# mbitsnbites/himg

Measured on AMD Instinct MI355X. Metric: Mpixels/s encode+decode, 4K RGBA q=50, higher is better.
Workload: dtype u8/i16/i32 integer

## Files before the change

himg_amd/csrc/himg_dev.h:

```cpp
#ifndef HIMG_DEV_H_
#define HIMG_DEV_H_

#include <hip/hip_runtime.h>
#include <stdint.h>

namespace himg_dev {

constexpr int kNumSym = 261;
constexpr int kHistStride = 264;
constexpr int kLresSpan = 16384;
constexpr int kIterSyms = 4096;
constexpr int kTreeStride = 384;
constexpr int kMaxCodeLen = 32;
constexpr int kHeadLen = 175;

struct Geom {
  int W, H, C, stride;
  int rows, cols, mrows, mcols;
  int chan_size, lres_size;
  int row_block;
  int ycbcr;
  int lres_spans;
  int use_blocks;
  int fix_t2;
// ... 105 lines not shown
static_assert(kRowTabWords % 4 == 0, "whole 16-byte words");

constexpr int kLresMemoWords = 6;
constexpr int kRecHdr = 72;
constexpr int kRecWin = 8;
struct DecWs {
  DecFrame *frames;
  uint32_t *nodes;
  uint2 *grp;
  uint32_t *gyc;
  uint2 *sub;
  uint32_t *row_off;
  uint32_t *row_len;
  uint8_t *lres_sym;         size_t lres_stride;
  uint8_t *fres_sym;         size_t fres_stride;
  uint8_t *low;              size_t plane_stride;
  uint32_t *lane_start;
  uint32_t *lane_off;
  uint32_t *lane_q;
  uint32_t *parse_stats;
  uint32_t *stats;
  uint32_t *rc_stats;
  int lres_chunks;
  uint32_t *spec_start;
  uint32_t *spec_endpos;
  uint32_t *spec_cnt;
  uint32_t *spec_memo;
  uint64_t *spec_end;
  uint64_t *fix_end;
  uint64_t *spec_tot;
  uint64_t *ver_base;
  int32_t *ver_ok;
  uint64_t *lres_endbit;
};


struct Profiler;

bool enc_uses_row_tokens(const Geom &g, int batch);
int enc_tok_seg(const Geom &g);
inline bool enc_tok_stage_fits(const Geom &g) { return tok_stage_need(g.row_block, enc_tok_seg(g)) <= kTokStage; }
void launch_tok_expand(const Geom &g, const EncWs &ws, int frame, uint8_t *dst, hipStream_t stream);

void launch_encode(const Geom &g, const EncWs &ws, int batch, const uint8_t *d_frames,
                   uint8_t *d_out, size_t out_stride, uint32_t *d_sizes,
                   const StaticChunks &sc, const ShiftTables &st, const LresTables &lt,
                   const uint8_t *d_fmap_lut, hipStream_t stream, Profiler *prof,
                   hipStream_t side, hipEvent_t ev_fork, hipEvent_t ev_join);

void enc_fill_qual_tab(const StaticChunks &sc, const ShiftTables &st, const LresTables &lt, QualTab *qt);
void launch_encode_q(const Geom &g, const EncWs &ws, int batch, const uint8_t *d_frames,
                     uint8_t *d_out, size_t out_stride, uint32_t *d_sizes,
                     const StaticChunks &sc, const QualSel &qs,
                     const uint8_t *d_fmap_lut, hipStream_t stream, Profiler *prof,
                     hipStream_t side, hipEvent_t ev_fork, hipEvent_t ev_join);
struct BudgetState {
  int32_t *quality;
  const uint32_t *budget;
  int32_t *lo, *hi;
  int32_t *state;
  int32_t *err;
};
enum { kBudgetSearch = 0, kBudgetFound = 1, kBudgetTooSmall = 2, kBudgetError = 3 };
void launch_budget_step(const BudgetState &bs, const EncWs &ws, int batch, int probe, int probes, int qmin, int qmax,
                        const uint32_t *d_sizes, int32_t *d_quality, hipStream_t stream, Profiler *prof);
void launch_budget_finish(const BudgetState &bs, const EncWs &ws, int batch, uint32_t *d_sizes, int32_t *d_status,
// ... 109 lines not shown
```

himg_amd/csrc/himg_hip.hip:

```cpp
#include "himg_hip.h"

#include <hip/hip_runtime.h>

#include <cmath>
#include <cstdio>
#include <cstdlib>
#include <cstring>
#include <string>
#include <vector>

#include "himg_dev.h"
#include "himg_tables.h"

using namespace himg_dev;

namespace himg_dev {

struct Profiler {
  bool enabled = false;
  struct Rec { const char *name; hipEvent_t a, b; };
  std::vector<Rec> pending;
  struct Acc { std::string name; double ms = 0; int n = 0; };
  std::vector<Acc> acc;
  const char *cur = nullptr;
// ... 505 lines not shown
      !ctx->d_grp.reserve((size_t)batch * 2 * (1u << kLutBits) * 8) ||
      !ctx->d_gyc.reserve((size_t)batch * 2 * (1u << kLutBits) * 4) ||
      !ctx->d_sub.reserve((size_t)batch * 2 * kSubEntries * 8) ||
      !ctx->d_lane.reserve((size_t)batch * g.rows * (2 * kDecThreads + himg_dev::kRecHdr + (region || himg_dev::dec_rows_fit_lds(g) ? 0 : 6 * kDecThreads)) * 4) ||
      !ctx->d_rows.reserve((size_t)batch * g.rows * 4 * 2) || !ctx->d_lres.reserve(lres * batch) ||
      (!region && !ctx->d_fres.reserve(fres * batch)) || !ctx->d_planes.reserve(plane * batch) ||
      !ctx->d_sizes.reserve((size_t)batch * (region ? 12 : 4)) ||
      !ctx->d_stats.reserve(((size_t)batch * (g.rows + 1) * 8 + (size_t)batch * 4 + (size_t)batch * g.rows * 8) * 4))
    return fail(ctx, HIMG_ERR_HIP, "decoder workspace allocation failed");
  w.frames = (DecFrame *)ctx->d_frames.p;
  w.nodes = (uint32_t *)ctx->d_nodes.p;
  w.grp = (uint2 *)ctx->d_grp.p;
  w.gyc = (uint32_t *)ctx->d_gyc.p;
  w.sub = (uint2 *)ctx->d_sub.p;
  w.lane_start = head_only ? nullptr : (uint32_t *)ctx->d_lane.p;
  w.lane_off = head_only ? nullptr : w.lane_start + (size_t)batch * g.rows * kDecThreads;
  w.lane_q = (head_only || region || himg_dev::dec_rows_fit_lds(g)) ? nullptr : w.lane_off + (size_t)batch * g.rows * (kDecThreads + himg_dev::kRecHdr);
  w.row_off = head_only ? nullptr : (uint32_t *)ctx->d_rows.p;
  w.row_len = head_only ? nullptr : w.row_off + (size_t)batch * g.rows;
  w.lres_sym = (uint8_t *)ctx->d_lres.p; w.lres_stride = lres;
  w.fres_sym = (head_only || region) ? nullptr : (uint8_t *)ctx->d_fres.p; w.fres_stride = (head_only || region) ? 0 : fres;
  w.low = (uint8_t *)ctx->d_planes.p; w.plane_stride = plane;
  w.stats = (uint32_t *)ctx->d_stats.p;
  w.parse_stats = w.stats + (size_t)batch * (g.rows + 1) * 8;
  w.rc_stats = head_only ? nullptr : w.parse_stats + (size_t)batch * 4;
  {
    const size_t max_bits = 8ull * ((size_t)g.lres_size + kTreeStride);
    const size_t cb = (size_t)kDecThreads * kLresSubBits;
    int nch = (int)((max_bits + cb - 1) / cb);
    if (nch > 1024) nch = 1024;
    w.lres_chunks = nch;
    size_t off = 0;
    auto carve = [&](size_t bytes) { size_t o = off; off += round_up(bytes, 256); return o; };
    const size_t o_ss = carve((size_t)batch * nch * kDecThreads * 4);
    const size_t o_sc = carve((size_t)batch * nch * kDecThreads * 4);
    const size_t o_se = carve((size_t)batch * nch * 8);
    const size_t o_st = carve((size_t)batch * nch * 8);
    const size_t o_sp = carve((size_t)batch * nch * kDecThreads * 4);
    const size_t o_fe = carve((size_t)batch * nch * 8);
    const size_t o_vb = carve((size_t)batch * nch * 8);
    const size_t o_ok = carve((size_t)batch * 4);
    const size_t o_eb = carve((size_t)batch * 8);
    const size_t o_mm = carve((size_t)batch * nch * kDecThreads * 4 * himg_dev::kLresMemoWords);
    if (!ctx->d_spec.reserve(off)) return fail(ctx, HIMG_ERR_HIP, "decoder workspace allocation failed");
    uint8_t *b = (uint8_t *)ctx->d_spec.p;
    w.spec_start = (uint32_t *)(b + o_ss); w.spec_cnt = (uint32_t *)(b + o_sc);
    w.spec_end = (uint64_t *)(b + o_se); w.spec_tot = (uint64_t *)(b + o_st);
    w.spec_endpos = (uint32_t *)(b + o_sp); w.fix_end = (uint64_t *)(b + o_fe);
    w.ver_base = (uint64_t *)(b + o_vb); w.ver_ok = (int32_t *)(b + o_ok);
    w.lres_endbit = (uint64_t *)(b + o_eb);
    w.spec_memo = (uint32_t *)(b + o_mm);
  }
  ctx->dec_geom = g;
  ctx->dec_batch = batch;
  ctx->dec_valid = true;
  return HIMG_OK;
}

static std::string format_message(int32_t st) {
  static const char *kStage[] = {"", "Not a RIFF HIMG file.\n", "Error decoding header.\n",
                                 "Error decoding low-res mapping function.\n",
                                 "Error decoding low-res data.\n",
                                 "Error decoding quantization configuration.\n",
                                 "Error decoding full-res mapping function.\n",
                                 "Error decoding full-res data.\n"};
  std::string m;
  if (st & 0x100) m += "Error: Invalid Huffman data.\n";
  const int stage = (st >> 4) & 7;
  m += kStage[stage];
  return m;
}

static int status_to_code(int32_t st) {
  st &= 15;
  switch (st) {
    case 0: return HIMG_OK;
    case 1: return HIMG_ERR_ARG;
    case 3: return HIMG_ERR_UNSUPPORTED;
// ... 1875 lines not shown
```

himg_amd/csrc/kernels_dec.hip:

```cpp
#include "himg_dev.h"
#include "loop_counts.h"

#include <cstdlib>
#include <type_traits>

namespace himg_dev {

__device__ static constexpr uint8_t kScanD[64] = {
    0,  1,  9,  8,  16, 17, 18, 10, 2,  3,  11, 19, 27, 26, 25, 24,
    32, 33, 34, 35, 36, 28, 20, 12, 4,  5,  13, 21, 29, 37, 45, 44,
    43, 42, 41, 40, 48, 49, 50, 51, 52, 53, 54, 46, 38, 30, 22, 14,
    6,  7,  15, 23, 31, 39, 47, 55, 63, 62, 61, 60, 59, 58, 57, 56};

__device__ static constexpr uint8_t kInvScanD[64] = {
    0, 1, 8, 9, 24, 25, 48, 49, 3, 2, 7, 10, 23, 26, 47, 50, 4, 5, 6, 11, 22, 27, 46, 51, 15, 14, 13, 12, 21, 28, 45, 52, 16, 17, 18, 19, 20, 29, 44, 53, 35, 34, 33, 32, 31, 30, 43, 54, 36, 37, 38, 39, 40, 41, 42, 55, 63, 62, 61, 60, 59, 58, 57, 56};

constexpr int kStGeom = 1, kStUnsupported = 3, kStFormat = 4;
__device__ __host__ constexpr int fmt_err(int stage, int huff) { return kStFormat | (stage << 4) | (huff << 8); }
constexpr int kMaxDepth = 32;
constexpr int kMaxNodes = 2 * kNumSym - 1;
constexpr int kMaxSlow = 128;

__device__ __forceinline__ int clamp255d(int x) { return x < 0 ? 0 : (x > 255 ? 255 : x); }

// ... 2333 lines not shown
}

template <bool FAST>
__global__ __launch_bounds__(256) void k_sse(Geom g, const uint8_t *frames, const uint8_t *fres_sym, size_t fres_stride,
                                             const uint8_t *rec, size_t plane_stride, const SseTab *tabs,
                                             const int32_t *quality, unsigned long long *sse) {
  __shared__ __attribute__((aligned(16))) uint32_t s_tab[kRowTabWords];
  __shared__ unsigned long long s_part[4];
  const int v = blockIdx.y, f = blockIdx.z, tid = threadIdx.x;
  const int q = __builtin_amdgcn_readfirstlane(
      ((const __attribute__((address_space(4))) int32_t *)(uintptr_t)quality)[f]);
  if (tid < kRowTabWords / 4) reinterpret_cast<uint4 *>(s_tab)[tid] = reinterpret_cast<const uint4 *>(tabs[q].w)[tid];
  __syncthreads();
  const int16_t *s_unmap = reinterpret_cast<const int16_t *>(s_tab);
  const uint8_t *s_shift = reinterpret_cast<const uint8_t *>(s_tab + 128);
  const uint32_t *s_shiftp = s_tab + 160;
  const int it = blockIdx.x * 256 + tid;
  uint32_t acc = 0;
  if (pair_tile(it) < g.cols)
    acc = transform_store_pair<(FAST ? -1 : 0), FAST, true>(
        g, g.cols, fres_sym + (size_t)f * fres_stride + (size_t)v * g.row_block, rec + (size_t)f * plane_stride,
        s_unmap, s_shift, s_shiftp, g.ycbcr, pair_tile(it), pair_half(it), v, nullptr, nullptr, true, false, 0,
        frames + (size_t)f * (size_t)g.frame_bytes, g.stride);
#pragma unroll
  for (int d = 32; d >= 1; d >>= 1) acc += __shfl_xor(acc, d);
  if ((tid & 63) == 0) s_part[tid >> 6] = acc;
  __syncthreads();
  if (tid == 0) {
    const unsigned long long t = s_part[0] + s_part[1] + s_part[2] + s_part[3];
    if (t) __hip_atomic_fetch_add(sse + f, t, __ATOMIC_RELAXED, __HIP_MEMORY_SCOPE_AGENT);
  }
}

template <int COLS, bool TENS = false>
__device__ __forceinline__ void dec_row_fused_body(const Geom &g, const DecWs &ws, const uint8_t *packed,
                                                   size_t in_stride, const uint32_t *sizes,
                                                   uint8_t *out_frames, int r0, int r1, int rpw,
                                                   const int bx, const int f, const int gx, const int gy,
                                                   const uint32_t next_lin, const bool again, const bool same_tables,
                                                   TensK td = nullptr) {
  extern __shared__ __attribute__((aligned(16))) uint8_t smem[];
  if (COLS == 512) rpw = 1;
  const FusedLayout L = fused_layout(g.row_block, rpw);
  const uint32_t rb16 = ((uint32_t)g.row_block + 15u) & ~15u;
  uint8_t *sym0 = smem + L.sym;
  LdsTables &T = *reinterpret_cast<LdsTables *>(smem + L.tab);
  StreamShared *sh = reinterpret_cast<StreamShared *>(smem + L.sh);
  int16_t *s_unmap = reinterpret_cast<int16_t *>(smem + L.unmap);
  uint8_t *s_shift = smem + L.shift;
  uint32_t *s_shiftp = reinterpret_cast<uint32_t *>(smem + L.shiftp);

  int tid_ = threadIdx.x;
  asm volatile("" : "+v"(tid_));
  __builtin_assume(tid_ >= 0 && tid_ < kDecThreads);
  const int tid = tid_;
  const long long c_in = clock64();
  DecFrame *df = ws.frames + f;
  const uint8_t *low = ws.low + (size_t)f * ws.plane_stride;
  PreLane pl = {};
  uint32_t pre_lr[4] = {0, 0, 0, 0}, pre_off0 = 0, pre_len0 = 0;
  if constexpr (COLS == 512) {
    const size_t ri = (size_t)f * g.rows + (size_t)(r0 + bx);
    const uint32_t *ps = ws.lane_start + ri * kDecThreads, *po = ws.lane_off + ri * (kDecThreads + kRecHdr);
    pl.start = ps[tid]; pl.off = po[tid]; pl.nxt = po[tid + 1];
    pl.nstart = tid + 1 < kDecThreads ? ps[tid + 1] : ~0u;
    pl.tot = po[kDecThreads]; pl.endrel = po[kDecThreads + 1]; pl.valid = po[kDecThreads + 2]; pl.rounds = po[kDecThreads + 3];
    pre_off0 = ws.row_off[ri]; pre_len0 = ws.row_len[ri];
    const int u = pair_tile(tid), hs = pair_half(tid), v = r0 + bx;
    const int u2 = min(u + 1, COLS - 1), v2 = min(v + 1, g.rows - 1);
    const uint32_t pstride = (uint32_t)g.rows * COLS, o1 = (uint32_t)v * COLS, o2 = (uint32_t)v2 * COLS;
#pragma unroll
    for (int cc = 0; cc < 2; ++cc) {
      const uint32_t m = (uint32_t)(2 * hs + cc) * pstride;
// ... 26 lines not shown
  const int rb = r0 + bx * rpw;
  const int nr = COLS == 512 ? 1 : min(rpw, r1 - rb);
  if (COLS == 512 && again) __syncthreads();
  {
    uint4 z;
    z.x = z.y = z.z = z.w = 0;
    const int n16 = (int)(rb16 >> 4) * nr;
    for (int k = tid; k < n16; k += kDecThreads) reinterpret_cast<uint4 *>(sym0)[k] = z;
  }
  if (ld_tab) {
    reinterpret_cast<uint4 *>(T.grp)[tid] = t_grp;
    if (tid < kRowTabWords / 4) reinterpret_cast<uint4 *>(smem + L.unmap)[tid] = t_row;
    if (tid < kSubEntries / 2) reinterpret_cast<uint4 *>(T.grp + (1 << kLutBits))[tid] = t_sub;
    if (tid < kMaxNodes + 1) T.nd[tid] = t_nd;
  }
  if constexpr (COLS == 512) {
    if (tid == 0) { sh->flag = st0; sh->err = 0; sh->endbit = ~0ull; }
  }
  __syncthreads();
  if constexpr (COLS == 512) {
    if (sh->flag) return;
  }

  auto decode_row = [&](int i) {
    const int r = rb + i;
    if (tid == 0) {
      uint32_t *st = ws.stats + ((size_t)f * (g.rows + 1) + r + 1) * 8;
      st[2] = 0; st[3] = 0;
    }
    if constexpr (COLS == 512) {
      uint32_t *st = ws.stats + ((size_t)f * (g.rows + 1) + r + 1) * 8;
      const int rc = decode_row_recorded(p, sizes[f], pre_off0, pre_len0, (uint32_t)g.row_block, tb, sh, sym0, st, pl);
      if (rc >= 0) return rc;
      return decode_stream_fused_cold(p, sizes[f], pre_off0, pre_len0, (uint32_t)g.row_block,
                                      reinterpret_cast<const uint32_t *>(tb.grp), tb.nd, sh, sym0, st,
                                      (uint32_t)g.max_sub, (uint32_t)g.lead_bits);
    }
    const size_t ri = (size_t)f * g.rows + (size_t)r;
    const uint32_t *ps = ws.lane_start + ri * kDecThreads, *po = ws.lane_off + ri * (kDecThreads + kRecHdr);
    PreLane q;
    q.start = ps[tid]; q.off = po[tid]; q.nxt = po[tid + 1];
    q.nstart = tid + 1 < kDecThreads ? ps[tid + 1] : ~0u;
    q.tot = po[kDecThreads]; q.endrel = po[kDecThreads + 1]; q.valid = po[kDecThreads + 2]; q.rounds = po[kDecThreads + 3];
    const uint32_t off_r = ws.row_off[ri], len_r = ws.row_len[ri];
    if (i > 0) __syncthreads();
    if (tid == 0) { sh->err = 0; sh->endbit = ~0ull; }
    __syncthreads();
    uint32_t *st = ws.stats + ((size_t)f * (g.rows + 1) + r + 1) * 8;
    const int rc = decode_row_recorded(p, sizes[f], off_r, len_r, (uint32_t)g.row_block, tb, sh, sym0 + (size_t)i * rb16, st, q);
    if (rc >= 0) return rc;
    return decode_stream_fused_cold(p, sizes[f], off_r, len_r, (uint32_t)g.row_block,
                                    reinterpret_cast<const uint32_t *>(tb.grp), tb.nd, sh, sym0 + (size_t)i * rb16, st,
                                    (uint32_t)g.max_sub, (uint32_t)g.lead_bits);
  };
  int bad = 0;
  if constexpr (COLS == 512) {
    bad = decode_row(0);
  } else {
#pragma unroll 1
    for (int i = 0; i < nr && !bad; ++i) bad = decode_row(i);
  }
  if (bad) {
    if (tid == 0) atomicMax(&df->status, fmt_err(7, 1));
    return;
  }

  const long long c_p2 = clock64();
  uint32_t pf_a = 0;
  bool pf_on = false;
  {
    const int fn = (int)(next_lin / (uint32_t)gx), rn = r0 + (int)(next_lin % (uint32_t)gx) * rpw;
    pf_on = g.prefetch_rows != 0 && fn < gy && rn < r1;
    if (pf_on) {
      const int wv = tid >> 6, ln = tid & 63;
      const uint32_t guess = COLS == 512 ? pre_len0 : (uint32_t)((unsigned long long)sizes[f] * (uint32_t)nr / (uint32_t)g.rows);
      const uint32_t o = 128u * (uint32_t)((wv - 1) * 64 + ln);
      if (wv >= 1 && wv <= 5 && o < guess + 256u) {
        const unsigned long long at = (unsigned long long)ws.row_off[(size_t)fn * g.rows + (size_t)rn] + o;
        if (at + 4ull <= (unsigned long long)sizes[fn]) {
          const uint8_t *a = packed + (size_t)fn * in_stride + at;
          const uint8_t *al = reinterpret_cast<const uint8_t *>(reinterpret_cast<uintptr_t>(a) & ~(uintptr_t)3);
          asm volatile("global_load_dword %0, %1, off" : "=v"(pf_a) : "v"(al) : "memory");
        }
      }
    }
  }
  const int ycbcr = df->ycbcr;
  const int cols = COLS > 0 ? COLS : g.cols;
  uint8_t *img;
  if constexpr (TENS) img = out_frames + (size_t)f * ((size_t)g.W * g.H * (size_t)(td->co * tens_elem_size(td->dtype)));
  else img = out_frames + (size_t)f * ((size_t)g.W * g.H * g.C);
  const int per_row = ((cols + 31) >> 5) * 64;
  HIMG_SPAN_BEGIN("dec.transform");
// ... 7 lines not shown
                                            nullptr, 0, td);
  }
  HIMG_SPAN_END("dec.transform");
  if constexpr (COLS != 512) {
    if (pf_on && tid >= per_row * nr) asm volatile("s_waitcnt vmcnt(0)" ::"v"(pf_a) : "memory");
  }
  if ((tid & 63) == 0) {
    const long long c_out = clock64();
    for (int i = 0; i < nr; ++i) {
      uint32_t *st = ws.stats + ((size_t)f * (g.rows + 1) + rb + i + 1) * 8;
      atomicMax(&st[2], (uint32_t)((c_out - c_p2) >> 4));
      atomicMax(&st[3], (uint32_t)((c_out - c_in) >> 4));
    }
  }
}


template <class W, class T>
__device__ __forceinline__ void karg_copy(T *dst, const __attribute__((address_space(4))) T *src) {
  static_assert(sizeof(T) % sizeof(W) == 0 && alignof(T) >= alignof(W), "whole words");
  const __attribute__((address_space(4))) W *sw = (const __attribute__((address_space(4))) W *)src;
  W *dw = reinterpret_cast<W *>(dst);
#pragma unroll
  for (size_t i = 0; i < sizeof(T) / sizeof(W); ++i) dw[i] = sw[i];
}
struct RowArgs {
  Geom g;
  DecWs ws;
  const uint8_t *packed;
  size_t in_stride;
  const uint32_t *sizes;
  uint8_t *out_frames;
  int r0, r1, rpw, gx, gy, next_dist;
};
template <int COLS>
__global__ __launch_bounds__(kDecThreads) void k_dec_row_fused(RowArgs) {
  typedef const __attribute__((address_space(4))) RowArgs *KArgs;
  KArgs ka = (KArgs)__builtin_amdgcn_kernarg_segment_ptr();
  const uint32_t total = (uint32_t)ka->gx * (uint32_t)ka->gy, S = gridDim.x;
  auto element = [&](uint32_t i) { return i * S + (blockIdx.x + 37u * i) % S; };
  bool again = false;
  int f_prev = -1;
#pragma unroll 1
  for (uint32_t i = 0; i * S < total; ++i) {
    const uint32_t lin = element(i);
    if (lin >= total) break;
    asm volatile("" : "+s"(ka));
    Geom g;
    DecWs ws;
    karg_copy<uint32_t>(&g, &ka->g);
    karg_copy<unsigned long long>(&ws, &ka->ws);
    const int gx = ka->gx, f = (int)(lin / (uint32_t)gx);
    const uint32_t nd = (uint32_t)ka->next_dist;
    dec_row_fused_body<COLS>(g, ws, ka->packed, ka->in_stride, ka->sizes, ka->out_frames, ka->r0, ka->r1, ka->rpw,
                             (int)(lin % (uint32_t)gx), f, gx, ka->gy, nd ? lin + nd : element(i + 1), again, f == f_prev);
    again = true;
    f_prev = f;
  }
}

struct RowArgsT {
  RowArgs a;
  TensDesc t;
};
template <int COLS>
__global__ __launch_bounds__(kDecThreads) void k_dec_row_fused_t(RowArgsT) {
  typedef const __attribute__((address_space(4))) RowArgsT *KArgs;
  KArgs ka = (KArgs)__builtin_amdgcn_kernarg_segment_ptr();
  const uint32_t total = (uint32_t)ka->a.gx * (uint32_t)ka->a.gy, S = gridDim.x;
  auto element = [&](uint32_t i) { return i * S + (blockIdx.x + 37u * i) % S; };
  bool again = false;
  int f_prev = -1;
#pragma unroll 1
  for (uint32_t i = 0; i * S < total; ++i) {
    const uint32_t lin = element(i);
    if (lin >= total) break;
    asm volatile("" : "+s"(ka));
    Geom g;
    DecWs ws;
    karg_copy<uint32_t>(&g, &ka->a.g);
    karg_copy<unsigned long long>(&ws, &ka->a.ws);
    const int gx = ka->a.gx, f = (int)(lin / (uint32_t)gx);
    const uint32_t nd = (uint32_t)ka->a.next_dist;
    dec_row_fused_body<COLS, true>(g, ws, ka->a.packed, ka->a.in_stride, ka->a.sizes, ka->a.out_frames, ka->a.r0,
                                   ka->a.r1, ka->a.rpw, (int)(lin % (uint32_t)gx), f, gx, ka->a.gy,
                                   nd ? lin + nd : element(i + 1), again, f == f_prev, &ka->t);
    again = true;
    f_prev = f;
  }
}

constexpr int kRowsPerCount = 4;

__device__ __forceinline__ uint32_t block_scan_u32d(uint32_t v, uint32_t *sm, uint32_t *total) {
  const int lane = threadIdx.x & 63, wave = threadIdx.x >> 6;
  uint32_t incl = v;
#pragma unroll
  for (int d = 1; d < 64; d <<= 1) {
    const uint32_t t = __shfl_up(incl, d);
    if (lane >= d) incl += t;
  }
  if (lane == 63) sm[wave] = incl;
  __syncthreads();
  uint32_t pre = 0, tot = 0;
#pragma unroll
  for (int w = 0; w < kDecThreads / 64; ++w) {
    const uint32_t x = sm[w];
    if (w < wave) pre += x;
    tot += x;
  }
  *total = tot;
  return pre + incl - v;
}

template <class RD, bool QTR = false>
__device__ __forceinline__ void row_count_one(RD &rd, const GrpTables &tb, StreamShared *sh, uint32_t *sm32,
                                              uint32_t rel0, uint32_t rem, uint32_t sb, uint32_t lead_bits,
                                              uint32_t *l_start, uint32_t *l_off, uint32_t *rc, long long c_in,
                                              uint32_t *l_q = nullptr, uint32_t out_size = 0, uint32_t window = 0) {
  const int tid = threadIdx.x;
  const uint32_t rel_end = rel0 + rem;
  const SubGrid sg = sub_grid(rel0, rem, sb, tid);
// ... 426 lines not shown
      if (touches || (exact && wi == (int)((out_size - 1u) / kRowWindow))) {
        uint32_t end_bp = ~0u;
        const uint32_t op = off - w0 + kWinGuard;
        if (inside) {
          if (!lean_write<true>(rd, tb, rel0 + st_rel, lim, op, win, span, usable == 3u)) sh.err = 1;
        } else if (exact) {
          if (!exact_write<true>(rd, tb, rel0 + st_rel, lim, op, rel_out, win, &end_bp, span)) sh.err = 1;
          if (end_bp != ~0u) sh.endbit = (unsigned long long)(end_bp - rel0);
        }
      }
    }
    const uint32_t qn = q - (uint32_t)tid + (uint32_t)kDecThreads;
    const int more = __syncthreads_or((tid == kDecThreads - 1 && q < nrec && nxt < w1) ? 1 : 0);
    if (!more || qn >= nrec) break;
    q = qn + (uint32_t)tid;
    st_rel = rec_pos(q); nst_rel = rec_pos(q + 1u); off = rec_off(q); nxt = rec_off(q + 1u);
  }
  __syncthreads();
  uint8_t *dst = ws.fres_sym + (size_t)f * ws.fres_stride + (size_t)r * g.row_block + w0;
  for (uint32_t k = tid; k < (w1 - w0) / 16u; k += kDecThreads)
    reinterpret_cast<uint4 *>(dst)[k] = reinterpret_cast<const uint4 *>(win + kWinGuard)[k];
  if (tid == 0 && w1 == out_size) {
    int bad = sh.err;
    if (tot < out_size) bad = 1;
    const unsigned long long E = sh.endbit;
    if (!bad && !(E <= P1 && E + 8 > P1 && E > 0)) bad = 1;
    if (bad) atomicMax(&df->status, fmt_err(7, 1));
  } else if (tid == 0 && sh.err) {
    atomicMax(&df->status, fmt_err(7, 1));
  }
}

__global__ __launch_bounds__(256) void k_dec_zero(uint4 *sym, uint32_t n16, uint32_t *a, uint32_t na, uint32_t *b,
                                                  uint32_t nb) {
  uint4 z;
  z.x = z.y = z.z = z.w = 0;
  const uint32_t k0 = blockIdx.x * (256u * 4u) + threadIdx.x;
#pragma unroll
  for (int j = 0; j < 4; ++j) {
    const uint32_t k = k0 + (uint32_t)j * 256u;
    if (k < n16) sym[k] = z;
  }
  const uint32_t stride_t = gridDim.x * 256u, t0 = blockIdx.x * 256u + threadIdx.x;
  for (uint32_t k = t0; k < na; k += stride_t) a[k] = 0;
  for (uint32_t k = t0; k < nb; k += stride_t) b[k] = 0;
}

__global__ void k_dec_status(DecWs ws, int32_t *status, int batch) {
  const int f = blockIdx.x * blockDim.x + threadIdx.x;
  if (f < batch) {
    const DecFrame *df = ws.frames + f;
    const int w = df->parse_status == 0 ? df->walk_status : 0;
    status[f] = df->status > w ? df->status : w;
  }
}

__device__ __forceinline__ void ycc_to_rgb(uint32_t &c0, uint32_t &c1, uint32_t &c2) {
  const int y = (int)c0, cb = ((int)c1 << 1) - 255, cr = ((int)c2 << 1) - 255;
  const int gg = y - ((cb + cr + 2) >> 2), b = gg + cb, r = gg + cr;
  c0 = (uint32_t)clamp255d(r); c1 = (uint32_t)clamp255d(gg); c2 = (uint32_t)clamp255d(b);
}

__global__ __launch_bounds__(256) void k_lres_preview(Geom g, DecWs ws, uint8_t *out) {
  const int f = blockIdx.y;
  const DecFrame *df = ws.frames + f;
  if (df->status) return;
  const uint32_t npix = (uint32_t)g.rows * (uint32_t)g.cols;
  const uint32_t p0 = 4u * (blockIdx.x * 256u + threadIdx.x);
  if (p0 >= npix) return;
  const int C = g.C, ycc = df->ycbcr;
  const uint8_t *plane = ws.low + (size_t)f * ws.plane_stride;
  uint8_t *dst = out + (size_t)f * npix * (uint32_t)C;
  const uint32_t np = npix - p0 < 4u ? npix - p0 : 4u;
  uint32_t v[4][4];
#pragma unroll
  for (int k = 0; k < 4; ++k)
#pragma unroll
    for (int c = 0; c < 4; ++c)
// ... 703 lines not shown
    return;
  }
  const uint8_t *low = ws.low + (size_t)f * ws.plane_stride;
  uint8_t *img = sa.out + (size_t)f * ((size_t)sa.h * sa.w * g.C);
  const int ycbcr = df->ycbcr;
#pragma unroll 1
  for (int ul = tid; ul < ww; ul += kDecThreads)
    scaled_tile_store_crop<S>(g, (int)L.seg, S * S * (int)L.seg, sym + 4 + ul, low, s_unmap, s_shift, ycbcr, su0 + ul,
                              r, rr, img);
}

#define HIMG_LAUNCH(name, grid, block, ...)                    \
  do {                                                         \
    prof_begin(prof, #name, stream);                           \
    hipLaunchKernelGGL(name, grid, block, 0, stream, __VA_ARGS__); \
    prof_end(prof, stream);                                    \
  } while (0)

int loop_counts_read_dec(unsigned long long *out) { return loop_counts_read(out); }

constexpr uint32_t kLdsMax = 160u * 1024u;
constexpr uint32_t kRowWindowLds = (uint32_t)sizeof(LdsTables) + 64u + kRowWindow + 2u * kWinGuard + 16u;

bool dec_rows_fit_lds(const Geom &g) { return fused_layout(g.row_block).total <= kLdsMax; }

hipError_t dec_set_kernel_attrs() {
  const void *fused[] = {reinterpret_cast<const void *>(&k_dec_row_fused<512>),
                         reinterpret_cast<const void *>(&k_dec_row_fused<256>),
                         reinterpret_cast<const void *>(&k_dec_row_fused<240>),
                         reinterpret_cast<const void *>(&k_dec_row_fused<-1>),
                         reinterpret_cast<const void *>(&k_dec_row_fused<0>),
                         reinterpret_cast<const void *>(&k_dec_row_fused_t<512>),
                         reinterpret_cast<const void *>(&k_dec_row_fused_t<-1>),
                         reinterpret_cast<const void *>(&k_dec_row_fused_t<0>)};
  for (const void *k : fused) {
    hipFuncAttributes fa;
    hipError_t e = hipFuncGetAttributes(&fa, k);
    if (e == hipSuccess)
      e = hipFuncSetAttribute(k, hipFuncAttributeMaxDynamicSharedMemorySize, (int)(kLdsMax - fa.sharedSizeBytes));
    if (e != hipSuccess) return e;
  }
  hipError_t e = hipFuncSetAttribute(reinterpret_cast<const void *>(&k_row_window), hipFuncAttributeMaxDynamicSharedMemorySize,
                                     (int)kRowWindowLds);
  if (e != hipSuccess) return e;
  hipFuncAttributes fa;
  e = hipFuncGetAttributes(&fa, reinterpret_cast<const void *>(&k_dec_region));
  if (e == hipSuccess)
    e = hipFuncSetAttribute(reinterpret_cast<const void *>(&k_dec_region), hipFuncAttributeMaxDynamicSharedMemorySize,
                            (int)(kLdsMax - fa.sharedSizeBytes));
  if (e == hipSuccess) e = hipFuncGetAttributes(&fa, reinterpret_cast<const void *>(&k_dec_region_t));
  if (e == hipSuccess)
    e = hipFuncSetAttribute(reinterpret_cast<const void *>(&k_dec_region_t), hipFuncAttributeMaxDynamicSharedMemorySize,
                            (int)(kLdsMax - fa.sharedSizeBytes));
  const void *scaled[] = {reinterpret_cast<const void *>(&k_dec_scaled<4, true>), reinterpret_cast<const void *>(&k_dec_scaled<2, true>),
                          reinterpret_cast<const void *>(&k_dec_scaled<4, false>), reinterpret_cast<const void *>(&k_dec_scaled<2, false>),
                          reinterpret_cast<const void *>(&k_dec_scaled_region<4>), reinterpret_cast<const void *>(&k_dec_scaled_region<2>)};
  for (const void *k : scaled) {
    if (e == hipSuccess) e = hipFuncGetAttributes(&fa, k);
    if (e == hipSuccess)
      e = hipFuncSetAttribute(k, hipFuncAttributeMaxDynamicSharedMemorySize, (int)(kLdsMax - fa.sharedSizeBytes));
  }
  return e;
}

int region_strip_tiles(const Geom &g) {
  const uint32_t fixed = region_layout(g.C, 0).total - region_layout(g.C, 0).seg * 64u * (uint32_t)g.C;
  const uint32_t seg = (kLdsMax - 1024u - fixed) / (64u * (uint32_t)g.C) & ~3u;
// ... 4 lines not shown
  const uint32_t nseg = (scale_log2 == 1 ? 16u : 4u) * (uint32_t)g.C;
  const RegionLayout L0 = scale_log2 == 1 ? scaled_layout<4>(g.C, 0) : scaled_layout<2>(g.C, 0);
  const uint32_t fixed = L0.total - L0.seg * nseg;
  const uint32_t seg = (kLdsMax - 1024u - fixed) / nseg & ~3u;
  return (int)(seg - 8u);
}

void launch_rowwalk_only(const Geom &g, const DecWs &ws, const uint8_t *d_packed, size_t in_stride,
                         const uint32_t *d_sizes, hipStream_t stream) {
  hipLaunchKernelGGL(k_dec_rowwalk, dim3(1), dim3(64), 0, stream, g, ws, d_packed, in_stride, d_sizes, 0x7fffffff, 0);
}

void launch_rowwalk_range(const Geom &g, const DecWs &ws, const uint8_t *d_packed, size_t in_stride,
                          const uint32_t *d_sizes, int row_end, bool resume, hipStream_t stream) {
  hipLaunchKernelGGL(k_dec_rowwalk, dim3(1), dim3(64), 0, stream, g, ws, d_packed, in_stride, d_sizes, row_end, resume ? 1 : 0);
}

static void launch_lres_chain(const Geom &g, const DecWs &ws, int batch, const uint8_t *d_packed, size_t in_stride,
                              const uint32_t *d_sizes, hipStream_t stream, Profiler *prof) {
  HIMG_LAUNCH(k_lres_spec, dim3(ws.lres_chunks, batch), dim3(kDecThreads), g, ws, d_packed, in_stride, d_sizes);
  HIMG_LAUNCH(k_lres_fix, dim3(batch), dim3(kDecThreads), g, ws, d_packed, in_stride, d_sizes);
  HIMG_LAUNCH(k_lres_write, dim3(ws.lres_chunks, batch), dim3(kDecThreads), g, ws, d_packed,
              in_stride, d_sizes);
  HIMG_LAUNCH(k_lres_finish, dim3((batch + 63) / 64), dim3(64), ws, batch);
  HIMG_LAUNCH(k_lres_unpredict, dim3((g.mcols + 4 * kUnpredWaves - 1) / (4 * kUnpredWaves), g.mrows, batch * g.C),
              dim3(64 * kUnpredWaves), g, ws);
}

static void launch_zero(const Geom &g, const DecWs &ws, int batch, hipStream_t stream, Profiler *prof) {
  const uint32_t n16 = (uint32_t)(((size_t)batch * ws.lres_stride + 15) / 16);
  const uint32_t ns = (uint32_t)((size_t)batch * (g.rows + 1) * 8), nr = ws.rc_stats ? (uint32_t)((size_t)batch * g.rows * 8) : 0u;
  prof_begin(prof, "memset", stream);
  hipLaunchKernelGGL(k_dec_zero, dim3((n16 + 256 * 4 - 1) / (256 * 4)), dim3(256), 0, stream,
                     reinterpret_cast<uint4 *>(ws.lres_sym), n16, ws.stats, ns, ws.rc_stats, nr);
  prof_end(prof, stream);
}

struct CountRule { bool wave; int rpc; Geom g; };
static CountRule count_rule(const Geom &g, long long all_rows, bool one_record) {
  CountRule c = {g.count_wave >= 0 ? g.count_wave != 0 : all_rows >= 8192,
                 all_rows <= 512 ? 1 : all_rows <= 1024 ? 2 : kRowsPerCount, g};
  if (one_record) c.g.max_sub = 0x7fffffff;
  return c;
}

void launch_preview(const Geom &g, const DecWs &ws, int batch, const uint8_t *d_packed, size_t in_stride,
                    const uint32_t *d_sizes, uint32_t *d_head_sizes, uint8_t *d_out, int32_t *d_status,
                    hipStream_t stream, Profiler *prof) {
  launch_zero(g, ws, batch, stream, prof);
  HIMG_LAUNCH(k_dec_parse_head, dim3(batch), dim3(kParseThreads), g, ws, d_packed, in_stride, d_sizes, d_head_sizes);
  launch_lres_chain(g, ws, batch, d_packed, in_stride, d_head_sizes, stream, prof);
  const uint32_t npix = (uint32_t)g.rows * (uint32_t)g.cols;
  HIMG_LAUNCH(k_lres_preview, dim3((npix + 1023u) / 1024u, batch), dim3(256), g, ws, d_out);
  HIMG_LAUNCH(k_dec_status, dim3((batch + 63) / 64), dim3(64), ws, d_status, batch);
}

struct WindowExtents { int nrows = 0, ntiles = 0; long long all_rows = 0; bool stop_early = false; };
static WindowExtents window_extents(const Geom &g, int batch, const int32_t *h_org, int S, int w, int h) {
  WindowExtents e;
  const int F = 8 / S;
  for (int f = 0; f < batch; ++f) {
    const int x = h_org[2 * f] / F, y = h_org[2 * f + 1] / F;
    const int r0 = y / S, r1 = (y + h + S - 1) / S, nt = (x + w + S - 1) / S - x / S;
    e.nrows = r1 - r0 > e.nrows ? r1 - r0 : e.nrows;
    e.ntiles = nt > e.ntiles ? nt : e.ntiles;
    e.stop_early |= r1 < g.rows;
    e.all_rows += r1 - r0;
// ... 212 lines not shown
      row_count(cnt_stream, seg_lo(k), seg_lo(k + 1));
      (void)hipEventRecord(ds->ev_cnt[k], cnt_stream);
      if (!wps) {
        hipStream_t ws_ = (nseg > 1 && ds->side3) ? ds->side3 : cnt_stream;
        if (ws_ != cnt_stream) (void)hipStreamWaitEvent(ws_, ds->ev_cnt[k], 0);
        window_pass(ws_, seg_lo(k), seg_lo(k + 1));
        (void)hipEventRecord(ds->ev_win[k], ws_);
      }
    }
  } else if (d_row_index) {
    HIMG_LAUNCH(k_dec_set_index, dim3(1), dim3(256), g, ws, d_row_index, d_sizes, r0, r1);
  } else {
    HIMG_LAUNCH(k_dec_rowwalk, dim3(batch), dim3(64), g, ws, d_packed, in_stride, d_sizes, kWalkAll, 0);
  }
  if (do_head) launch_lres_chain(g, ws, batch, d_packed, in_stride, d_sizes, stream, prof);
  if (!do_rows) return;
  if (wps) {
    const int per_row = ((g.cols + 31) / 32) * 64;
    int rpw = 1;
    while (rpw < 8 && (rpw + 1) * per_row <= kDecThreads && fused_layout(g.row_block, rpw + 1).total <= kLdsMax) ++rpw;
    if (g.W == 4096 && g.C == 4 && (g.H & 7) == 0) rpw = 1;
    const uint32_t lds = fused_layout(g.row_block, rpw).total;
    const int n_cu = ho.n_cu, per_cu = 1;
#define HIMG_FUSED_LAUNCH(COLS, A, B)                                                           \
  do {                                                                                          \
    const int gx_ = ((B) - (A) + rpw - 1) / rpw;                                                \
    const long long all_ = (long long)gx_ * batch;                                              \
    const int slots_ = ho.persist_rows > 1 ? ho.persist_rows : n_cu * per_cu;                   \
    const bool pers_ = ho.persist_rows != 0 && all_ > slots_;                                   \
    RowArgs ra_;                                                                                \
    ra_.g = g; ra_.ws = ws; ra_.packed = d_packed; ra_.in_stride = in_stride; ra_.sizes = d_sizes; \
    ra_.out_frames = d_out; ra_.r0 = (A); ra_.r1 = (B); ra_.rpw = rpw; ra_.gx = gx_; ra_.gy = batch; \
    ra_.next_dist = pers_ ? 0 : n_cu * per_cu;                                                 \
    if (tens) {                                                                                 \
      RowArgsT rt_;                                                                             \
      rt_.a = ra_; rt_.t = *tens;                                                               \
      hipLaunchKernelGGL((k_dec_row_fused_t<(COLS) == 256 || (COLS) == 240 ? -1 : (COLS)>),     \
                         dim3((unsigned)(pers_ ? slots_ : all_)), dim3(kDecThreads), lds, stream, rt_); \
    } else                                                                                      \
    hipLaunchKernelGGL((k_dec_row_fused<COLS>), dim3((unsigned)(pers_ ? slots_ : all_)),        \
                       dim3(kDecThreads), lds, stream, ra_);                                    \
  } while (0)
    for (int k = 0; k < nseg; ++k) {
      const int a = seg_lo(k), b = seg_lo(k + 1);
      if (ds) (void)hipStreamWaitEvent(stream, ds->ev_cnt[k], 0);
      else row_count(stream, a, b);
      if (b <= a) continue;
      const bool whole4 = g.C == 4 && (g.W & 7) == 0 && (g.H & 7) == 0;
      prof_begin(prof, !tens ? "k_dec_row_fused" : g.W == 4096 && whole4 ? "k_dec_row_fused_t<512>"
                                                 : whole4 ? "k_dec_row_fused_t<-1>" : "k_dec_row_fused_t<0>", stream);
      if (g.W == 4096 && whole4) HIMG_FUSED_LAUNCH(512, a, b);
      else if (g.W == 2048 && whole4) HIMG_FUSED_LAUNCH(256, a, b);
      else if (g.W == 1920 && whole4) HIMG_FUSED_LAUNCH(240, a, b);
      else if (whole4) HIMG_FUSED_LAUNCH(-1, a, b);
      else HIMG_FUSED_LAUNCH(0, a, b);
      prof_end(prof, stream);
    }
#undef HIMG_FUSED_LAUNCH
  } else {
    for (int k = 0; k < nseg; ++k) {
      const int a = seg_lo(k), b = seg_lo(k + 1);
      if (ds) (void)hipStreamWaitEvent(stream, ds->ev_win[k], 0);
      else { row_count(stream, a, b); window_pass(stream, a, b); }
      if (b <= a) continue;
      if (tens) {
        TileArgsT ta;
        ta.g = g; ta.ws = ws; ta.out_frames = d_out; ta.v0 = a; ta.t = *tens;
        if (g.C == 4 && (g.W & 7) == 0 && (g.H & 7) == 0) HIMG_LAUNCH(k_tile_inv_t<true>, dim3(gx, b - a, batch), dim3(256), ta);
        else HIMG_LAUNCH(k_tile_inv_t<false>, dim3(gx, b - a, batch), dim3(256), ta);
      } else
      if (g.C == 4 && (g.W & 7) == 0 && (g.H & 7) == 0) HIMG_LAUNCH(k_tile_inv<true>, dim3(gx, b - a, batch), dim3(256), g, ws, d_out, a);
      else HIMG_LAUNCH(k_tile_inv<false>, dim3(gx, b - a, batch), dim3(256), g, ws, d_out, a);
    }
  }
  HIMG_LAUNCH(k_dec_status, dim3((batch + 63) / 64), dim3(64), ws, d_status, batch);
// ... 49 lines not shown
```

Measured before the change: 100,200.

## Split cold Huffman decode fallback into separate deferred kernel

Removes the slow-path stream decoder from the fused row kernel. Row groups whose recorded decode fails are pushed to a global cold list, and a follow-up kernel launched after each segment decodes them. The aim is to cut register and code pressure in the hot fused kernel so it reaches higher occupancy. The cost is an extra kernel launch per segment plus atomics and list workspace, and the cold kernel relaunches the full body for failed rows.

```diff
diff --git a/himg_amd/csrc/himg_dev.h b/himg_amd/csrc/himg_dev.h
--- a/himg_amd/csrc/himg_dev.h
+++ b/himg_amd/csrc/himg_dev.h
@@ -161,6 +161,8 @@
   uint64_t *ver_base;
   int32_t *ver_ok;
   uint64_t *lres_endbit;
+  uint32_t *cold_cnt;
+  uint32_t *cold_list;
 };
 
 
diff --git a/himg_amd/csrc/himg_hip.hip b/himg_amd/csrc/himg_hip.hip
--- a/himg_amd/csrc/himg_hip.hip
+++ b/himg_amd/csrc/himg_hip.hip
@@ -561,6 +561,7 @@
     w.lres_chunks = nch;
     size_t off = 0;
     auto carve = [&](size_t bytes) { size_t o = off; off += round_up(bytes, 256); return o; };
+    const size_t o_cc = carve(2 * himg_dev::kWalkSegs * 4);
     const size_t o_ss = carve((size_t)batch * nch * kDecThreads * 4);
     const size_t o_sc = carve((size_t)batch * nch * kDecThreads * 4);
     const size_t o_se = carve((size_t)batch * nch * 8);
@@ -571,8 +572,13 @@
     const size_t o_ok = carve((size_t)batch * 4);
     const size_t o_eb = carve((size_t)batch * 8);
     const size_t o_mm = carve((size_t)batch * nch * kDecThreads * 4 * himg_dev::kLresMemoWords);
+    const size_t o_cl = carve(((size_t)batch * g.rows + himg_dev::kWalkSegs) * 4);
+    const void *spec_was = ctx->d_spec.p;
     if (!ctx->d_spec.reserve(off)) return fail(ctx, HIMG_ERR_HIP, "decoder workspace allocation failed");
     uint8_t *b = (uint8_t *)ctx->d_spec.p;
+    if (b != spec_was && hipMemset(b + o_cc, 0, 2 * himg_dev::kWalkSegs * 4) != hipSuccess)
+      return fail(ctx, HIMG_ERR_HIP, "decoder workspace allocation failed");
+    w.cold_cnt = (uint32_t *)(b + o_cc); w.cold_list = (uint32_t *)(b + o_cl);
     w.spec_start = (uint32_t *)(b + o_ss); w.spec_cnt = (uint32_t *)(b + o_sc);
     w.spec_end = (uint64_t *)(b + o_se); w.spec_tot = (uint64_t *)(b + o_st);
     w.spec_endpos = (uint32_t *)(b + o_sp); w.fix_end = (uint64_t *)(b + o_fe);
diff --git a/himg_amd/csrc/kernels_dec.hip b/himg_amd/csrc/kernels_dec.hip
--- a/himg_amd/csrc/kernels_dec.hip
+++ b/himg_amd/csrc/kernels_dec.hip
@@ -2389,13 +2389,13 @@
   }
 }
 
-template <int COLS, bool TENS = false>
+template <int COLS, bool TENS = false, bool COLD = false>
 __device__ __forceinline__ void dec_row_fused_body(const Geom &g, const DecWs &ws, const uint8_t *packed,
                                                    size_t in_stride, const uint32_t *sizes,
                                                    uint8_t *out_frames, int r0, int r1, int rpw,
                                                    const int bx, const int f, const int gx, const int gy,
                                                    const uint32_t next_lin, const bool again, const bool same_tables,
-                                                   TensK td = nullptr) {
+                                                   const int cold_k, const uint32_t cold_base, TensK td = nullptr) {
   extern __shared__ __attribute__((aligned(16))) uint8_t smem[];
   if (COLS == 512) rpw = 1;
   const FusedLayout L = fused_layout(g.row_block, rpw);
@@ -2488,9 +2488,10 @@
       uint32_t *st = ws.stats + ((size_t)f * (g.rows + 1) + r + 1) * 8;
       const int rc = decode_row_recorded(p, sizes[f], pre_off0, pre_len0, (uint32_t)g.row_block, tb, sh, sym0, st, pl);
       if (rc >= 0) return rc;
-      return decode_stream_fused_cold(p, sizes[f], pre_off0, pre_len0, (uint32_t)g.row_block,
-                                      reinterpret_cast<const uint32_t *>(tb.grp), tb.nd, sh, sym0, st,
-                                      (uint32_t)g.max_sub, (uint32_t)g.lead_bits);
+      if constexpr (!COLD) return -1;
+      else return decode_stream_fused_cold(p, sizes[f], pre_off0, pre_len0, (uint32_t)g.row_block,
+                                           reinterpret_cast<const uint32_t *>(tb.grp), tb.nd, sh, sym0, st,
+                                           (uint32_t)g.max_sub, (uint32_t)g.lead_bits);
     }
     const size_t ri = (size_t)f * g.rows + (size_t)r;
     const uint32_t *ps = ws.lane_start + ri * kDecThreads, *po = ws.lane_off + ri * (kDecThreads + kRecHdr);
@@ -2505,9 +2506,10 @@
     uint32_t *st = ws.stats + ((size_t)f * (g.rows + 1) + r + 1) * 8;
     const int rc = decode_row_recorded(p, sizes[f], off_r, len_r, (uint32_t)g.row_block, tb, sh, sym0 + (size_t)i * rb16, st, q);
     if (rc >= 0) return rc;
-    return decode_stream_fused_cold(p, sizes[f], off_r, len_r, (uint32_t)g.row_block,
-                                    reinterpret_cast<const uint32_t *>(tb.grp), tb.nd, sh, sym0 + (size_t)i * rb16, st,
-                                    (uint32_t)g.max_sub, (uint32_t)g.lead_bits);
+    if constexpr (!COLD) return -1;
+    else return decode_stream_fused_cold(p, sizes[f], off_r, len_r, (uint32_t)g.row_block,
+                                         reinterpret_cast<const uint32_t *>(tb.grp), tb.nd, sh, sym0 + (size_t)i * rb16, st,
+                                         (uint32_t)g.max_sub, (uint32_t)g.lead_bits);
   };
   int bad = 0;
   if constexpr (COLS == 512) {
@@ -2515,6 +2517,10 @@
   } else {
 #pragma unroll 1
     for (int i = 0; i < nr && !bad; ++i) bad = decode_row(i);
+  }
+  if (!COLD && bad < 0) {
+    if (tid == 0) ws.cold_list[cold_base + atomicAdd(&ws.cold_cnt[2 * cold_k], 1u)] = (uint32_t)f * (uint32_t)gx + (uint32_t)bx;
+    return;
   }
   if (bad) {
     if (tid == 0) atomicMax(&df->status, fmt_err(7, 1));
@@ -2588,6 +2594,8 @@
   const uint32_t *sizes;
   uint8_t *out_frames;
   int r0, r1, rpw, gx, gy, next_dist;
+  int cold_k;
+  uint32_t cold_base;
 };
 template <int COLS>
 __global__ __launch_bounds__(kDecThreads) void k_dec_row_fused(RowArgs) {
@@ -2609,7 +2617,8 @@
     const int gx = ka->gx, f = (int)(lin / (uint32_t)gx);
     const uint32_t nd = (uint32_t)ka->next_dist;
     dec_row_fused_body<COLS>(g, ws, ka->packed, ka->in_stride, ka->sizes, ka->out_frames, ka->r0, ka->r1, ka->rpw,
-                             (int)(lin % (uint32_t)gx), f, gx, ka->gy, nd ? lin + nd : element(i + 1), again, f == f_prev);
+                             (int)(lin % (uint32_t)gx), f, gx, ka->gy, nd ? lin + nd : element(i + 1), again, f == f_prev,
+                             ka->cold_k, ka->cold_base);
     again = true;
     f_prev = f;
   }
@@ -2640,10 +2649,49 @@
     const uint32_t nd = (uint32_t)ka->a.next_dist;
     dec_row_fused_body<COLS, true>(g, ws, ka->a.packed, ka->a.in_stride, ka->a.sizes, ka->a.out_frames, ka->a.r0,
                                    ka->a.r1, ka->a.rpw, (int)(lin % (uint32_t)gx), f, gx, ka->a.gy,
-                                   nd ? lin + nd : element(i + 1), again, f == f_prev, &ka->t);
+                                   nd ? lin + nd : element(i + 1), again, f == f_prev, ka->a.cold_k, ka->a.cold_base, &ka->t);
     again = true;
     f_prev = f;
   }
+}
+
+template <int COLS, bool TENS, class KA>
+__device__ __forceinline__ void dec_row_cold_loop(KA ka, TensK td) {
+  const uint32_t *cnt = ka->ws.cold_cnt + 2 * ka->cold_k;
+  const uint32_t n = __hip_atomic_load(cnt, __ATOMIC_RELAXED, __HIP_MEMORY_SCOPE_AGENT);
+  const uint32_t total = (uint32_t)ka->gx * (uint32_t)ka->gy;
+  bool again = false;
+#pragma unroll 1
+  for (uint32_t i = blockIdx.x; i < n; i += gridDim.x) {
+    asm volatile("" : "+s"(ka));
+    Geom g;
+    DecWs ws;
+    karg_copy<uint32_t>(&g, &ka->g);
+    karg_copy<unsigned long long>(&ws, &ka->ws);
+    const uint32_t lin = ws.cold_list[ka->cold_base + i];
+    if (lin >= total) continue;
+    const int gx = ka->gx;
+    dec_row_fused_body<COLS, TENS, true>(g, ws, ka->packed, ka->in_stride, ka->sizes, ka->out_frames, ka->r0, ka->r1, ka->rpw,
+                                         (int)(lin % (uint32_t)gx), (int)(lin / (uint32_t)gx), gx, ka->gy, total, again, false,
+                                         ka->cold_k, ka->cold_base, td);
+    again = true;
+  }
+  __syncthreads();
+  if (threadIdx.x == 0) {
+    uint32_t *c = ka->ws.cold_cnt + 2 * ka->cold_k;
+    if (atomicAdd(&c[1], 1u) == gridDim.x - 1u) { c[1] = 0; __hip_atomic_store(&c[0], 0u, __ATOMIC_RELAXED, __HIP_MEMORY_SCOPE_AGENT); }
+  }
+}
+template <int COLS>
+__global__ __launch_bounds__(kDecThreads) void k_dec_row_cold(RowArgs) {
+  typedef const __attribute__((address_space(4))) RowArgs *KArgs;
+  dec_row_cold_loop<COLS, false>((KArgs)__builtin_amdgcn_kernarg_segment_ptr(), nullptr);
+}
+template <int COLS>
+__global__ __launch_bounds__(kDecThreads) void k_dec_row_cold_t(RowArgsT) {
+  typedef const __attribute__((address_space(4))) RowArgsT *KArgs;
+  KArgs ka = (KArgs)__builtin_amdgcn_kernarg_segment_ptr();
+  dec_row_cold_loop<COLS, true>(&ka->a, &ka->t);
 }
 
 constexpr int kRowsPerCount = 4;
@@ -3136,7 +3184,7 @@
 }
 
 __global__ __launch_bounds__(256) void k_dec_zero(uint4 *sym, uint32_t n16, uint32_t *a, uint32_t na, uint32_t *b,
-                                                  uint32_t nb) {
+                                                  uint32_t nb, uint32_t *c, uint32_t nc) {
   uint4 z;
   z.x = z.y = z.z = z.w = 0;
   const uint32_t k0 = blockIdx.x * (256u * 4u) + threadIdx.x;
@@ -3148,6 +3196,7 @@
   const uint32_t stride_t = gridDim.x * 256u, t0 = blockIdx.x * 256u + threadIdx.x;
   for (uint32_t k = t0; k < na; k += stride_t) a[k] = 0;
   for (uint32_t k = t0; k < nb; k += stride_t) b[k] = 0;
+  for (uint32_t k = t0; k < nc; k += stride_t) c[k] = 0;
 }
 
 __global__ void k_dec_status(DecWs ws, int32_t *status, int batch) {
@@ -3917,7 +3966,11 @@
                          reinterpret_cast<const void *>(&k_dec_row_fused<0>),
                          reinterpret_cast<const void *>(&k_dec_row_fused_t<512>),
                          reinterpret_cast<const void *>(&k_dec_row_fused_t<-1>),
-                         reinterpret_cast<const void *>(&k_dec_row_fused_t<0>)};
+                         reinterpret_cast<const void *>(&k_dec_row_fused_t<0>),
+                         reinterpret_cast<const void *>(&k_dec_row_cold<-1>),
+                         reinterpret_cast<const void *>(&k_dec_row_cold<0>),
+                         reinterpret_cast<const void *>(&k_dec_row_cold_t<-1>),
+                         reinterpret_cast<const void *>(&k_dec_row_cold_t<0>)};
   for (const void *k : fused) {
     hipFuncAttributes fa;
     hipError_t e = hipFuncGetAttributes(&fa, k);
@@ -3988,7 +4041,7 @@
   const uint32_t ns = (uint32_t)((size_t)batch * (g.rows + 1) * 8), nr = ws.rc_stats ? (uint32_t)((size_t)batch * g.rows * 8) : 0u;
   prof_begin(prof, "memset", stream);
   hipLaunchKernelGGL(k_dec_zero, dim3((n16 + 256 * 4 - 1) / (256 * 4)), dim3(256), 0, stream,
-                     reinterpret_cast<uint4 *>(ws.lres_sym), n16, ws.stats, ns, ws.rc_stats, nr);
+                     reinterpret_cast<uint4 *>(ws.lres_sym), n16, ws.stats, ns, ws.rc_stats, nr, ws.cold_cnt, 2u * kWalkSegs);
   prof_end(prof, stream);
 }
 
@@ -4267,15 +4320,29 @@
     ra_.g = g; ra_.ws = ws; ra_.packed = d_packed; ra_.in_stride = in_stride; ra_.sizes = d_sizes; \
     ra_.out_frames = d_out; ra_.r0 = (A); ra_.r1 = (B); ra_.rpw = rpw; ra_.gx = gx_; ra_.gy = batch; \
     ra_.next_dist = pers_ ? 0 : n_cu * per_cu;                                                 \
+    ra_.cold_k = k; ra_.cold_base = cold_base;                                                  \
+    cold_base += (uint32_t)all_;                                                                \
+                 \
+    const unsigned cold_grid_ = (unsigned)(all_ < n_cu ? all_ : n_cu);                          \
     if (tens) {                                                                                 \
       RowArgsT rt_;                                                                             \
       rt_.a = ra_; rt_.t = *tens;                                                               \
       hipLaunchKernelGGL((k_dec_row_fused_t<(COLS) == 256 || (COLS) == 240 ? -1 : (COLS)>),     \
                          dim3((unsigned)(pers_ ? slots_ : all_)), dim3(kDecThreads), lds, stream, rt_); \
-    } else                                                                                      \
-    hipLaunchKernelGGL((k_dec_row_fused<COLS>), dim3((unsigned)(pers_ ? slots_ : all_)),        \
-                       dim3(kDecThreads), lds, stream, ra_);                                    \
+      prof_end(prof, stream);                                                                   \
+      prof_begin(prof, "k_dec_row_cold_t", stream);                                             \
+      if ((COLS) != 0) hipLaunchKernelGGL((k_dec_row_cold_t<-1>), dim3(cold_grid_), dim3(kDecThreads), lds, stream, rt_); \
+      else hipLaunchKernelGGL((k_dec_row_cold_t<0>), dim3(cold_grid_), dim3(kDecThreads), lds, stream, rt_); \
+    } else {                                                                                    \
+      hipLaunchKernelGGL((k_dec_row_fused<COLS>), dim3((unsigned)(pers_ ? slots_ : all_)),      \
+                         dim3(kDecThreads), lds, stream, ra_);                                  \
+      prof_end(prof, stream);                                                                   \
+      prof_begin(prof, "k_dec_row_cold", stream);                                               \
+      if ((COLS) != 0) hipLaunchKernelGGL((k_dec_row_cold<-1>), dim3(cold_grid_), dim3(kDecThreads), lds, stream, ra_); \
+      else hipLaunchKernelGGL((k_dec_row_cold<0>), dim3(cold_grid_), dim3(kDecThreads), lds, stream, ra_); \
+    }                                                                                           \
   } while (0)
+    uint32_t cold_base = 0;
     for (int k = 0; k < nseg; ++k) {
       const int a = seg_lo(k), b = seg_lo(k + 1);
       if (ds) (void)hipStreamWaitEvent(stream, ds->ev_cnt[k], 0);
```

After: 100,100. About the same (-0.0%).
